# mayuelala/FollowYourClick

Measured on NVIDIA H100. Metric: frames/sec (64x64x16f latent, 25 DDIM steps), higher is better.
Workload: dtype bf16

## Files before the change

### followyourclick_b200/csrc/gemm_tc.cu

```cuda
#include "tma.cuh"
#include "wgmma.cuh"

namespace {

constexpr int BM = 128;
constexpr int BK = 64;
constexpr int STAGES = 4;
constexpr int A_BYTES = BM * BK * 2;
constexpr int MAX_STAGES = 8;
constexpr int MAX_RING_BYTES = 192 * 1024;
constexpr int SMEM_LIMIT = 232448;
constexpr int SMEM_EXTRA = 256 + 1024;
constexpr int OUT_BOX_BYTES = 32;
constexpr int OUT_BOX_SMEM = 64 * OUT_BOX_BYTES;
constexpr int NUM_THREADS = 288;

struct TcParams {
  int64_t M;
  int N, N_out;
  int taps, cin_blocks;
  int BN, n_tiles;
  int bw, bh, bn, Wo, Ho, w_tiles, h_tiles;
  int lg_bw, lg_bh;
  int64_t m_tiles;
  int tap_dy[9], tap_dx[9], tap_img[9];
  const float* bias; const float* rowbias;
  int64_t rows_per_group;
  int64_t ldrb;
  float alpha;
  int flags;
  int cb_split;
  const float* ln_rs;
  int resident, a_stages;
  int ring_bytes, stg_bytes;
  int half_dw, half_dh, half_dn;
};

__device__ __forceinline__ void warpgroup_sync(int wg) {
  if (wg == 0) asm volatile("bar.sync 1, 128;" ::: "memory");
  else asm volatile("bar.sync 2, 128;" ::: "memory");
}

struct TileCoord { int n, w, h, i; };
__device__ __forceinline__ TileCoord tile_coord(const TcParams& p, int64_t t) {
  TileCoord c;
  const uint32_t tile = (uint32_t)t;
  c.n = (int)(tile % (uint32_t)p.n_tiles);
  const uint32_t m_blk = tile / (uint32_t)p.n_tiles;
  c.w = (int)(m_blk % (uint32_t)p.w_tiles);
  const uint32_t m2 = m_blk / (uint32_t)p.w_tiles;
  c.h = (int)(m2 % (uint32_t)p.h_tiles);
  c.i = (int)(m2 / (uint32_t)p.h_tiles);
  return c;
}

__device__ __forceinline__ int64_t tile_pixel(const TcParams& p, const TileCoord& c, int r) {
  const int ow = c.w * p.bw + (r & (p.bw - 1)), oh = c.h * p.bh + ((r >> p.lg_bw) & (p.bh - 1));
  const int img = c.i * p.bn + (r >> (p.lg_bw + p.lg_bh));
  const int64_t pix = ((int64_t)img * p.Ho + oh) * p.Wo + ow;
  return ((ow < p.Wo) && (oh < p.Ho) && (pix < p.M)) ? pix : -1;
}

__device__ __forceinline__ uint32_t stage_off(int row, int col, int esize) {
  const int cpb = OUT_BOX_BYTES / esize;
  const uint32_t in_box = (uint32_t)(row * OUT_BOX_BYTES + (col % cpb) * esize);
  return (uint32_t)(col / cpb) * OUT_BOX_SMEM + (in_box ^ (((in_box >> 7) & 1u) << 4));
}

template <int BN, typename T>
__device__ __forceinline__ void epilogue(const TcParams& p, const TileCoord& c, const float* acc, int wg, int warp4, int lane, uint8_t* stg) {
  const int q = lane & 3;
  const int flags = p.flags;
  const bool geglu = flags & FYC_EPI_GEGLU, out_f32 = flags & FYC_EPI_OUT_F32, lnf = flags & FYC_EPI_LNFOLD;
  const bool has_bias = flags & FYC_EPI_BIAS, has_res = flags & FYC_EPI_RESIDUAL, has_rb = flags & FYC_EPI_ROWBIAS;
#pragma unroll
  for (int half = 0; half < 2; ++half) {
    const int row = warp4 * 16 + (lane >> 2) + 8 * half;
    const int64_t pix = tile_pixel(p, c, wg * 64 + row);
    if (pix < 0) continue;
    const float rs = lnf ? __ldg(p.ln_rs + pix) : 1.0f;
    const float* rb = has_rb ? p.rowbias + (pix / p.rows_per_group) * p.ldrb : nullptr;
    if (geglu) {
      if constexpr (BN == 256) {
        const float* bp = p.bias + c.n * 256;
#pragma unroll
        for (int j = 0; j < 16; ++j) {
          const int col = 8 * j + 2 * q;
          if (c.n * 128 + col >= p.N_out) continue;
          const float2 ba = __ldg(reinterpret_cast<const float2*>(bp + col)), bg = __ldg(reinterpret_cast<const float2*>(bp + 128 + col));
          const float a0 = acc[4 * j + 2 * half], a1 = acc[4 * j + 2 * half + 1];
          const float g0 = acc[4 * (j + 16) + 2 * half], g1 = acc[4 * (j + 16) + 2 * half + 1];
          const float x = fmaf(a0, rs, ba.x) * gelu_erf_fast(fmaf(g0, rs, bg.x));
          const float y = fmaf(a1, rs, ba.y) * gelu_erf_fast(fmaf(g1, rs, bg.y));
          *reinterpret_cast<typename Pair16<T>::type*>(stg + stage_off(row, col, 2)) = Pair16<T>::pack(x, y);
        }
      }
      continue;
    }
    const float scale = lnf ? rs : p.alpha;
#pragma unroll
    for (int j = 0; j < BN / 8; ++j) {
      const int col = 8 * j + 2 * q, n = c.n * BN + col;
      if (n >= p.N) continue;
      float x = acc[4 * j + 2 * half] * scale, y = acc[4 * j + 2 * half + 1] * scale;
      if (has_bias) { const float2 b = __ldg(reinterpret_cast<const float2*>(p.bias + n)); x += b.x; y += b.y; }
      if (has_rb) { const float2 b = __ldg(reinterpret_cast<const float2*>(rb + n)); x += b.x; y += b.y; }
      if (out_f32) {
        float2* s = reinterpret_cast<float2*>(stg + stage_off(row, col, 4));
        if (has_res) { const float2 r = *s; x += r.x; y += r.y; }
        *s = make_float2(x, y);
      } else {
        typename Pair16<T>::type* s = reinterpret_cast<typename Pair16<T>::type*>(stg + stage_off(row, col, 2));
        if (has_res) { const float2 r = Pair16<T>::unpack(*s); x += r.x; y += r.y; }
        *s = Pair16<T>::pack(x, y);
      }
    }
  }
}

template <int BN, typename T>
__global__ void __launch_bounds__(NUM_THREADS, 1)
gemm_tc_kernel(const __grid_constant__ CUtensorMap map_a, const __grid_constant__ CUtensorMap map_w, const __grid_constant__ CUtensorMap map_a2,
               const __grid_constant__ CUtensorMap map_out, const __grid_constant__ CUtensorMap map_res, const TcParams p) {
  extern __shared__ __align__(1024) uint8_t smem_raw[];
  uint8_t* smem = smem_raw + pad1024(smem_raw);
  uint64_t* bars = reinterpret_cast<uint64_t*>(smem + p.ring_bytes + 2 * p.stg_bytes);
  uint64_t* full = bars;
  uint64_t* empty = bars + MAX_STAGES;
  uint64_t* wbar = bars + 2 * MAX_STAGES;
  uint64_t* rbar = wbar + 1;
  const int nstages = p.a_stages;
  const uint32_t slab_kb = (uint32_t)BN * (BK * 2);
  const uint32_t a_base = p.resident ? (uint32_t)(p.taps * p.cin_blocks) * slab_kb : 0u;
  const uint32_t a_stride = p.resident ? (uint32_t)A_BYTES : (uint32_t)A_BYTES + slab_kb;
  const int warp = threadIdx.x >> 5, lane = threadIdx.x & 31;
  const int k_iters = p.taps * p.cin_blocks;
  const int64_t num_tiles = p.m_tiles * p.n_tiles;

  if (threadIdx.x == 0) {
    for (int s = 0; s < MAX_STAGES; ++s) { mbar_init(&full[s], 1); mbar_init(&empty[s], 256); }
    mbar_init(wbar, 1);
    mbar_init(&rbar[0], 1); mbar_init(&rbar[1], 1);
    mbar_init_fence();
  }
  __syncthreads();

  if (warp == 8) {
    if (lane == 0) {
      asm volatile("prefetch.tensormap [%0];" ::"l"(reinterpret_cast<uint64_t>(&map_a)) : "memory");
      asm volatile("prefetch.tensormap [%0];" ::"l"(reinterpret_cast<uint64_t>(&map_w)) : "memory");
      asm volatile("prefetch.tensormap [%0];" ::"l"(reinterpret_cast<uint64_t>(&map_a2)) : "memory");
      int stage = 0; uint32_t phase = 0;
      const uint32_t tx_bytes = p.resident ? (uint32_t)A_BYTES : A_BYTES + slab_kb;
      if (p.resident) {
        const int n_blk = (int)(blockIdx.x % p.n_tiles);
        mbar_expect_tx(wbar, (uint32_t)k_iters * slab_kb);
        for (int k = 0; k < k_iters; ++k)
          tma_load_3d(&map_w, wbar, smem + (uint32_t)k * slab_kb, (k % p.cin_blocks) * BK, k / p.cin_blocks, n_blk * BN);
      }
      for (int64_t tile = blockIdx.x; tile < num_tiles; tile += gridDim.x) {
        const TileCoord tc = tile_coord(p, tile);
        const int ow0 = tc.w * p.bw, oh0 = tc.h * p.bh, img0 = tc.i * p.bn;
        for (int tap = 0; tap < p.taps; ++tap) {
          for (int cb = 0; cb < p.cin_blocks; ++cb) {
            mbar_wait(&empty[stage], phase ^ 1);
            uint8_t* sa = smem + a_base + (uint32_t)stage * a_stride;
            const bool seg2 = cb >= p.cb_split;
            const CUtensorMap* ma = seg2 ? &map_a2 : &map_a;
            const int ka = (seg2 ? cb - p.cb_split : cb) * BK;
            mbar_expect_tx(&full[stage], tx_bytes);
            tma_load_4d(ma, &full[stage], sa, ka, ow0 + p.tap_dx[tap], oh0 + p.tap_dy[tap], img0 + p.tap_img[tap]);
            if (!p.resident) tma_load_3d(&map_w, &full[stage], sa + A_BYTES, cb * BK, tap, tc.n * BN);
            if (++stage == nstages) { stage = 0; phase ^= 1; }
          }
        }
      }
    }
    return;
  }
  const int wg = warp >> 2, warp4 = warp & 3;
  const bool elected = (threadIdx.x & 127) == 0;
  auto stg = [&]() { return smem + p.ring_bytes + wg * p.stg_bytes; };
  const bool has_res = p.flags & FYC_EPI_RESIDUAL;
  auto cpb = [&]() { return (p.flags & FYC_EPI_OUT_F32) ? OUT_BOX_BYTES / 4 : OUT_BOX_BYTES / 2; };
  if (elected) {
    asm volatile("prefetch.tensormap [%0];" ::"l"(reinterpret_cast<uint64_t>(&map_out)) : "memory");
    if (has_res) asm volatile("prefetch.tensormap [%0];" ::"l"(reinterpret_cast<uint64_t>(&map_res)) : "memory");
  }
  float acc[BN / 2];
  int stage = 0; uint32_t phase = 0, rphase = 0;
  if (p.resident) mbar_wait(wbar, 0);
  auto half_tile = [&](int64_t t, int& col0, int& nbox, int& bw0, int& bh0, int& bn0) {
    const TileCoord tc = tile_coord(p, t);
    const int bn_out = (p.flags & FYC_EPI_GEGLU) ? BN / 2 : BN;
    col0 = tc.n * bn_out;
    nbox = min(bn_out, p.N_out - col0) / cpb();
    bw0 = tc.w * p.bw + wg * p.half_dw; bh0 = tc.h * p.bh + wg * p.half_dh; bn0 = tc.i * p.bn + wg * p.half_dn;
    return tile_pixel(p, tc, wg * 64) >= 0;
  };
  for (int64_t tile = blockIdx.x; tile < num_tiles; tile += gridDim.x) {
    if (has_res && elected) {
      int col0, nbox, bw0, bh0, bn0;
      if (half_tile(tile, col0, nbox, bw0, bh0, bn0)) {
        bulk_wait_read();
        mbar_expect_tx(&rbar[wg], (uint32_t)(nbox * OUT_BOX_SMEM));
        for (int b = 0; b < nbox; ++b) tma_load_4d(&map_res, &rbar[wg], stg() + b * OUT_BOX_SMEM, col0 + b * cpb(), bw0, bh0, bn0);
      }
    }
    int prev = -1;
    for (int k = 0; k < k_iters; ++k) {
      mbar_wait(&full[stage], phase);
      const uint32_t sa = smem_u32(smem + a_base + (uint32_t)stage * a_stride) + (uint32_t)wg * (64 * BK * 2);
      const uint64_t a_desc = wgmma_desc_sw128(sa);
      const uint64_t b_desc = wgmma_desc_sw128(p.resident ? smem_u32(smem) + (uint32_t)k * slab_kb : smem_u32(smem + (uint32_t)stage * a_stride) + A_BYTES);
      wgmma_fence();
#pragma unroll
      for (int kk = 0; kk < BK / 16; ++kk)
        Wgmma<BN, T>::ss(acc, a_desc + (uint64_t)(2 * kk), b_desc + (uint64_t)(2 * kk), (k > 0 || kk > 0) ? 1 : 0);
      wgmma_commit();
      wgmma_wait<1>();
      if (prev >= 0) mbar_arrive(&empty[prev]);
      prev = stage;
      if (++stage == nstages) { stage = 0; phase ^= 1; }
    }
    wgmma_wait<0>();
    wgmma_fence_regs<BN / 2>(acc);
    mbar_arrive(&empty[prev]);
    int col0, nbox, bw0, bh0, bn0;
    if (!half_tile(tile, col0, nbox, bw0, bh0, bn0)) continue;
    if (elected) bulk_wait_read();
    warpgroup_sync(wg);
    if (has_res) { mbar_wait(&rbar[wg], rphase); rphase ^= 1; }
    epilogue<BN, T>(p, tile_coord(p, tile), acc, wg, warp4, lane, stg());
    fence_async_smem();
    warpgroup_sync(wg);
    if (elected) {
      for (int b = 0; b < nbox; ++b) tma_store_4d(&map_out, stg() + b * OUT_BOX_SMEM, col0 + b * cpb(), bw0, bh0, bn0);
      bulk_commit();
    }
  }
  if (elected) bulk_wait_all();
}

__global__ void space_to_planes_kernel(const bf16* __restrict__ x, bf16* __restrict__ out, int64_t NB, int64_t H, int64_t W, int64_t C) {
  const int64_t cv = C / 8, H2 = H / 2, W2 = W / 2;
  const int64_t total = NB * H * W * cv;
  for (int64_t i = blockIdx.x * (int64_t)blockDim.x + threadIdx.x; i < total; i += (int64_t)gridDim.x * blockDim.x) {
    int64_t c = (i % cv) * 8; int64_t t = i / cv;
    int64_t w = t % W; t /= W;
    int64_t h = t % H; int64_t n = t / H;
    int64_t plane = 2 * (h & 1) + (w & 1);
    bf16* dst = out + ((((plane * NB + n) * H2) + h / 2) * W2 + w / 2) * C + c;
    *reinterpret_cast<uint4*>(dst) = *reinterpret_cast<const uint4*>(x + i * 8);
  }
}

int32_t encode_out_map(CUtensorMap* m, const void* base, const TcParams& p, int32_t dt, uint64_t cols, uint64_t W, uint64_t H, uint64_t NB,
                       uint64_t sw, uint64_t sh, uint64_t sn) {
  const bool f32 = (p.flags & FYC_EPI_OUT_F32) != 0;
  const uint64_t es = f32 ? 4 : 2;
  uint64_t dims[4] = {cols, W, H, NB};
  uint64_t str[3] = {sw * es, sh * es, sn * es};
  uint32_t box[4] = {(uint32_t)(OUT_BOX_BYTES / es), (uint32_t)(p.half_dw ? p.half_dw : p.bw), (uint32_t)(p.half_dh ? p.half_dh : p.bh),
                     (uint32_t)(p.half_dn ? p.half_dn : p.bn)};
  return encode_map(m, base, 4, dims, str, box, f32 ? CU_TENSOR_MAP_DATA_TYPE_FLOAT32 : tma_dtype(dt),
                    CU_TENSOR_MAP_SWIZZLE_32B);
}

constexpr int BN_CHOICES[] = {256, 192, 160, 128, 96, 80, 64, 48, 32, 16};
constexpr int MAX_BN_F32 = 128;

int pick_bn(int64_t N, bool geglu, bool f32) {
  if (geglu) return 256;
  for (int bn : BN_CHOICES)
    if (N % bn == 0 && (!f32 || bn <= MAX_BN_F32)) return bn;
  return 16;
}

int stg_bytes_for(int bn, int flags) {
  const int bn_out = (flags & FYC_EPI_GEGLU) ? bn / 2 : bn;
  return 64 * bn_out * ((flags & FYC_EPI_OUT_F32) ? 4 : 2);
}
int ring_bytes_for(int bn, int flags) {
  const int avail = (SMEM_LIMIT - SMEM_EXTRA - 2 * stg_bytes_for(bn, flags)) & ~1023;
  return avail < MAX_RING_BYTES ? avail : MAX_RING_BYTES;
}

void choose_tiles(TcParams& p, int* grid_out) {
  const int sms = fyc_sm_count();
  const bool geglu = (p.flags & FYC_EPI_GEGLU) != 0, f32 = (p.flags & FYC_EPI_OUT_F32) != 0;
  const int max_bn = f32 ? MAX_BN_F32 : 256;
  const int k_iters = p.taps * p.cin_blocks;
  p.resident = 0;
  p.BN = pick_bn(p.N, geglu, f32);
  p.n_tiles = (int)ceil_div64(p.N, p.BN);
  p.half_dw = p.half_dh = p.half_dn = 0;
  if (p.bn >= 2) p.half_dn = p.bn / 2;
  else if (p.bh >= 2) p.half_dh = p.bh / 2;
  else p.half_dw = p.bw / 2;
  int grid = 0;
  if (!geglu) {
    int rbn = 0;
    for (int min_stages = 4; min_stages >= 3 && !rbn; --min_stages)
      for (int bn : BN_CHOICES)
        if (bn >= 128 && bn <= max_bn && p.N % bn == 0 &&
            (int64_t)k_iters * bn * 128 <= ring_bytes_for(bn, p.flags) - min_stages * A_BYTES) { rbn = bn; break; }
    if (rbn) {
      const int nt = p.N / rbn;
      const int rgrid = (sms / nt) * nt;
      if (nt <= sms && rgrid * 16 >= sms * 15 && p.m_tiles * nt >= (int64_t)rgrid * 4) {
        p.resident = 1; p.BN = rbn; p.n_tiles = nt;
        grid = rgrid;
      }
    }
    const int64_t rounds0 = ceil_div64(p.m_tiles * p.n_tiles, sms);
    if (!p.resident && rounds0 < 8) {
      auto cost_of = [&](int bn, int64_t nt) {
        const int64_t mma = 8 * bn, feed = (int64_t)(5.3 * (128 + bn));
        return ceil_div64(p.m_tiles * nt, sms) * ((mma > feed ? mma : feed) + 400);
      };
      int64_t best = cost_of(p.BN, p.n_tiles);
      for (int bn : BN_CHOICES) {
        if (bn > p.N || bn < 64 || bn > max_bn) continue;
        const int64_t nt = ceil_div64(p.N, bn);
        const int64_t cost = cost_of(bn, nt);
        if (cost < best) { best = cost; p.BN = bn; p.n_tiles = (int)nt; }
      }
    }
  }
  p.stg_bytes = stg_bytes_for(p.BN, p.flags);
  p.ring_bytes = ring_bytes_for(p.BN, p.flags);
  const int slab = k_iters * p.BN * 128;
  const int st = p.resident ? (p.ring_bytes - slab) / A_BYTES : p.ring_bytes / (A_BYTES + p.BN * 128);
  p.a_stages = st > (p.resident ? MAX_STAGES : STAGES) ? (p.resident ? MAX_STAGES : STAGES) : st;
  if (!p.resident) {
    const int64_t tiles = p.m_tiles * p.n_tiles;
    grid = (int)(tiles < sms ? tiles : sms);
  }
  *grid_out = grid;
}

template <int BN, typename T>
int32_t launch_bn(const CUtensorMap& ma, const CUtensorMap& mw, const CUtensorMap& ma2, const CUtensorMap& mo, const CUtensorMap& mr,
                  const TcParams& p, int grid, cudaStream_t st) {
  static bool attr_set = false;
  if (!attr_set) {
    FYC_CUDA(cudaFuncSetAttribute(gemm_tc_kernel<BN, T>, cudaFuncAttributeMaxDynamicSharedMemorySize, SMEM_LIMIT));
    attr_set = true;
  }
  const int smem = p.ring_bytes + 2 * p.stg_bytes + SMEM_EXTRA;
  FYC_CHECK(smem <= SMEM_LIMIT && p.a_stages >= 2 && p.a_stages <= MAX_STAGES, "tensor-core GEMM: shared-memory plan does not fit (BN %d)", BN);
  gemm_tc_kernel<BN, T><<<grid, NUM_THREADS, smem, st>>>(ma, mw, ma2, mo, mr, p);
  FYC_LAUNCH_CHECK();
  return FYC_OK;
}

int32_t launch_tc(int32_t dt, const CUtensorMap& ma, const CUtensorMap& mw, const CUtensorMap& mo, const CUtensorMap* mr, TcParams p, int grid,
                  cudaStream_t st, const CUtensorMap* ma2p = nullptr) {
  const CUtensorMap& ma2 = ma2p ? *ma2p : ma;
  const CUtensorMap& mres = mr ? *mr : mo;
  if (!ma2p) p.cb_split = 0x7fffffff;
  FYC_CHECK(!(p.flags & FYC_EPI_RESIDUAL) || mr, "tensor-core GEMM: residual epilogue without a residual map");
  FYC_CHECK((p.bw & (p.bw - 1)) == 0 && (p.bh & (p.bh - 1)) == 0 && p.bw > 0 && p.bh > 0, "tensor-core GEMM: patch dims must be powers of two");
  p.lg_bw = 0; while ((1 << p.lg_bw) < p.bw) ++p.lg_bw;
  p.lg_bh = 0; while ((1 << p.lg_bh) < p.bh) ++p.lg_bh;
  const int64_t tiles = p.m_tiles * p.n_tiles;
  FYC_CHECK(tiles < (1ll << 31) && p.M < (1ll << 31) && p.rows_per_group < (1ll << 31), "tensor-core GEMM: problem exceeds the 32-bit tile index range");
  if (grid > tiles) grid = (int)tiles;
  FYC_DISPATCH16(dt, switch (p.BN) {
    case 256: return launch_bn<256, T>(ma, mw, ma2, mo, mres, p, grid, st);
    case 192: return launch_bn<192, T>(ma, mw, ma2, mo, mres, p, grid, st);
    case 160: return launch_bn<160, T>(ma, mw, ma2, mo, mres, p, grid, st);
    case 128: return launch_bn<128, T>(ma, mw, ma2, mo, mres, p, grid, st);
    case 96: return launch_bn<96, T>(ma, mw, ma2, mo, mres, p, grid, st);
    case 80: return launch_bn<80, T>(ma, mw, ma2, mo, mres, p, grid, st);
    case 64: return launch_bn<64, T>(ma, mw, ma2, mo, mres, p, grid, st);
    case 48: return launch_bn<48, T>(ma, mw, ma2, mo, mres, p, grid, st);
    case 32: return launch_bn<32, T>(ma, mw, ma2, mo, mres, p, grid, st);
    case 16: return launch_bn<16, T>(ma, mw, ma2, mo, mres, p, grid, st);
  })
  FYC_CHECK(false, "tensor-core GEMM: no kernel for BN = %d", p.BN);
}

}

bool fyc_gemm_tc_eligible(const fyc_gemm_args* g) {
  if (!fyc_is_16bit(g->dtype)) return false;
  if (g->K % 8 || g->lda % 8 || g->ldw % 8 || g->N % 16 || g->M < 64) return false;
  if (((uintptr_t)g->A | (uintptr_t)g->W) & 15) return false;
  if (g->batch > 1 && ((g->strideA | g->strideW | g->strideO) % 8)) return false;
  const int64_t n_out = (g->epilogue & FYC_EPI_GEGLU) ? g->N / 2 : g->N;
  if (g->ldo % 8 || ((uintptr_t)g->out & 15)) return false;
  if ((g->epilogue & FYC_EPI_RESIDUAL) && (g->ldr % 8 || ((uintptr_t)g->residual & 15))) return false;
  if ((g->epilogue & FYC_EPI_GEGLU) && (g->N % 256 || !(g->epilogue & FYC_EPI_BIAS) || (g->epilogue & ~(FYC_EPI_GEGLU | FYC_EPI_BIAS | FYC_EPI_LNFOLD)))) return false;
  if (g->A2) {
    if (g->batch != 1 || g->K1 <= 0 || g->K1 >= g->K || g->K1 % BK || g->lda2 % 8 || (((uintptr_t)g->A2) & 15)) return false;
  }
  if (g->epilogue & FYC_EPI_LNFOLD) {
    if (!g->ln_rowstats || (((uintptr_t)g->ln_rowstats) & 3)) return false;
    if (g->alpha != 1.0f || (g->epilogue & (FYC_EPI_OUT_F32 | FYC_EPI_RESIDUAL)) || g->N % 8) return false;
    if ((g->epilogue & FYC_EPI_ROWBIAS) && g->rows_per_group % 128) return false;
  }
  if ((g->epilogue & FYC_EPI_BIAS) && ((uintptr_t)g->bias & 15)) return false;
  if ((g->epilogue & FYC_EPI_ROWBIAS) && ((uintptr_t)g->rowbias & 15)) return false;
  (void)n_out;
  return tma_available();
}

int32_t fyc_gemm_tc(const fyc_gemm_args* g, cudaStream_t st) {
  FYC_CHECK(fyc_gemm_tc_eligible(g), "gemm(tensor cores): shape/alignment not eligible (M=%lld N=%lld K=%lld)", (long long)g->M,
            (long long)g->N, (long long)g->K);
  const bool geglu = (g->epilogue & FYC_EPI_GEGLU) != 0;
  const bool f32 = (g->epilogue & FYC_EPI_OUT_F32) != 0;
  for (int64_t b = 0; b < g->batch; ++b) {
    const uint16_t* A = (const uint16_t*)g->A + b * g->strideA;
    const uint16_t* W = (const uint16_t*)g->W + b * g->strideW;
    CUtensorMap ma, mw, ma2;
    const int64_t Ka = g->A2 ? g->K1 : g->K;
    {
      uint64_t dims[4] = {(uint64_t)Ka, (uint64_t)g->M, 1, 1};
      uint64_t str[3] = {(uint64_t)g->lda * 2, (uint64_t)g->lda * 2 * (uint64_t)g->M, (uint64_t)g->lda * 2 * (uint64_t)g->M};
      uint32_t box[4] = {BK, BM, 1, 1};
      int32_t rc = encode_map(&ma, A, 4, dims, str, box, tma_dtype(g->dtype));
      if (rc) return rc;
    }
    if (g->A2) {
      uint64_t dims[4] = {(uint64_t)(g->K - g->K1), (uint64_t)g->M, 1, 1};
      uint64_t str[3] = {(uint64_t)g->lda2 * 2, (uint64_t)g->lda2 * 2 * (uint64_t)g->M, (uint64_t)g->lda2 * 2 * (uint64_t)g->M};
      uint32_t box[4] = {BK, BM, 1, 1};
      int32_t rc = encode_map(&ma2, g->A2, 4, dims, str, box, tma_dtype(g->dtype));
      if (rc) return rc;
    }
    TcParams p{};
    p.M = g->M; p.N = (int)g->N; p.N_out = geglu ? (int)g->N / 2 : (int)g->N;
    p.taps = 1; p.cin_blocks = (int)ceil_div64(g->K, BK);
    p.bw = BM; p.bh = 1; p.bn = 1; p.Wo = (int)g->M; p.Ho = 1;
    p.w_tiles = (int)ceil_div64(g->M, BM); p.h_tiles = 1; p.m_tiles = p.w_tiles;
    p.flags = g->epilogue;
    int grid = 0;
    choose_tiles(p, &grid);
    p.tap_dy[0] = p.tap_dx[0] = p.tap_img[0] = 0;
    {
      uint64_t dims[3] = {(uint64_t)g->K, 1, (uint64_t)g->N};
      uint64_t str[2] = {(uint64_t)g->ldw * 2, (uint64_t)g->ldw * 2};
      uint32_t box[3] = {BK, 1, (uint32_t)p.BN};
      int32_t rc = encode_map(&mw, W, 3, dims, str, box, tma_dtype(g->dtype));
      if (rc) return rc;
    }
    FYC_CHECK(g->M < (1ll << 31), "gemm(tensor cores): M too large");
    p.bias = g->bias; p.rowbias = g->rowbias; p.rows_per_group = g->rows_per_group > 0 ? g->rows_per_group : 1; p.ldrb = g->N;
    p.alpha = g->alpha;
    p.ln_rs = g->ln_rowstats;
    p.cb_split = g->A2 ? (int)(g->K1 / BK) : 0x7fffffff;
    const int64_t es = f32 ? 4 : 2;
    const uint64_t M = (uint64_t)g->M, No = (uint64_t)p.N_out;
    CUtensorMap mo, mr;
    int32_t rc = encode_out_map(&mo, (const char*)g->out + b * g->strideO * es, p, g->dtype, No, M, 1, 1, g->ldo, g->ldo * M, g->ldo * M);
    if (rc) return rc;
    if (g->epilogue & FYC_EPI_RESIDUAL) {
      rc = encode_out_map(&mr, (const char*)g->residual + b * g->strideO * es, p, g->dtype, No, M, 1, 1, g->ldr, g->ldr * M, g->ldr * M);
      if (rc) return rc;
    }
    rc = launch_tc(g->dtype, ma, mw, mo, (g->epilogue & FYC_EPI_RESIDUAL) ? &mr : nullptr, p, grid, st, g->A2 ? &ma2 : nullptr);
    if (rc) return rc;
  }
  return FYC_OK;
}

static bool pick_patch(int64_t NB, int64_t Ho, int64_t Wo, int* bw, int* bh, int* bn) {
  int w = 1; while (w < 128 && Wo % (w * 2) == 0) w *= 2;
  int h = 1; while (w * h < 128 && Ho % (h * 2) == 0) h *= 2;
  int n = 128 / (w * h);
  if (w * h * n != 128 || NB % n != 0) return false;
  *bw = w; *bh = h; *bn = n;
  return true;
}

bool fyc_conv3x3_tc_eligible(const fyc_conv3x3_args* c) {
  if (!fyc_is_16bit(c->dtype) || c->upsample != 1) return false;
  if (c->stride != 1 && c->stride != 2) return false;
  if (c->Cin % 8 || c->Cout % 16) return false;
  if (c->stride == 2 && (c->H % 2 || c->W % 2)) return false;
  if (((uintptr_t)c->x | (uintptr_t)c->w | (uintptr_t)c->out) & 15) return false;
  if ((c->epilogue & FYC_EPI_RESIDUAL) && ((uintptr_t)c->residual & 15)) return false;
  if ((c->epilogue & FYC_EPI_ROWBIAS) && (((uintptr_t)c->rowbias & 15) || (c->ld_rowbias > 0 && c->ld_rowbias % 4))) return false;
  if (c->epilogue & FYC_EPI_GEGLU) return false;
  int bw, bh, bn;
  if (!pick_patch(c->NB, c->H / c->stride, c->W / c->stride, &bw, &bh, &bn)) return false;
  return tma_available();
}

int32_t fyc_conv3x3_tc(const fyc_conv3x3_args* c, const void* x_planes, cudaStream_t st) {
  FYC_CHECK(fyc_conv3x3_tc_eligible(c), "conv3x3(tensor cores): shape/alignment not eligible");
  const int s = c->stride;
  const int64_t Ho = c->H / s, Wo = c->W / s;
  TcParams p{};
  pick_patch(c->NB, Ho, Wo, &p.bw, &p.bh, &p.bn);
  p.M = c->NB * Ho * Wo; p.N = (int)c->Cout; p.N_out = p.N;
// ... 115 lines not shown
```

### followyourclick_b200/csrc/wgmma.cuh

```cuda
#pragma once
#include <stdint.h>

#include "common.cuh"

template <int N, typename T = bf16> struct Wgmma;

#define FYC_WGMMA_16(T, TY) \
template <> struct Wgmma<16, T> { \
  static __device__ __forceinline__ void ss(float* d, uint64_t da, uint64_t db, int scale_d) { \
    asm volatile("{\n.reg .pred p;\nsetp.ne.b32 p, %10, 0;\n" \
                 "wgmma.mma_async.sync.aligned.m64n16k16.f32." TY "." TY " {%0, %1, %2, %3, %4, %5, %6, %7}, %8, %9, p, 1, 1, 0, 0;\n}" \
                 : "+f"(d[0]), "+f"(d[1]), "+f"(d[2]), "+f"(d[3]), "+f"(d[4]), "+f"(d[5]), "+f"(d[6]), "+f"(d[7]) \
                 : "l"(da), "l"(db), "r"(scale_d)); \
  } \
};
FYC_WGMMA_16(bf16, "bf16")
FYC_WGMMA_16(f16, "f16")
#undef FYC_WGMMA_16

#define FYC_WGMMA_32(T, TY) \
template <> struct Wgmma<32, T> { \
  static __device__ __forceinline__ void ss(float* d, uint64_t da, uint64_t db, int scale_d) { \
    asm volatile("{\n.reg .pred p;\nsetp.ne.b32 p, %18, 0;\n" \
                 "wgmma.mma_async.sync.aligned.m64n32k16.f32." TY "." TY " {%0, %1, %2, %3, %4, %5, %6, %7, %8, %9, %10, %11, %12, %13, %14, %15}, %16, %17, p, 1, 1, 0, 0;\n}" \
// ... 85 lines not shown
  } \
};
FYC_WGMMA_128(bf16, "bf16")
FYC_WGMMA_128(f16, "f16")
#undef FYC_WGMMA_128

#define FYC_WGMMA_160(T, TY) \
template <> struct Wgmma<160, T> { \
  static __device__ __forceinline__ void ss(float* d, uint64_t da, uint64_t db, int scale_d) { \
    asm volatile("{\n.reg .pred p;\nsetp.ne.b32 p, %82, 0;\n" \
                 "wgmma.mma_async.sync.aligned.m64n160k16.f32." TY "." TY " {%0, %1, %2, %3, %4, %5, %6, %7, %8, %9, %10, %11, %12, %13, %14, %15, %16, %17, %18, %19, %20, %21, %22, %23, %24, %25, %26, %27, %28, %29, %30, %31, %32, %33, %34, %35, %36, %37, %38, %39, %40, %41, %42, %43, %44, %45, %46, %47, %48, %49, %50, %51, %52, %53, %54, %55, %56, %57, %58, %59, %60, %61, %62, %63, %64, %65, %66, %67, %68, %69, %70, %71, %72, %73, %74, %75, %76, %77, %78, %79}, %80, %81, p, 1, 1, 0, 0;\n}" \
                 : "+f"(d[0]), "+f"(d[1]), "+f"(d[2]), "+f"(d[3]), "+f"(d[4]), "+f"(d[5]), "+f"(d[6]), "+f"(d[7]), "+f"(d[8]), "+f"(d[9]), "+f"(d[10]), "+f"(d[11]), "+f"(d[12]), "+f"(d[13]), "+f"(d[14]), "+f"(d[15]), "+f"(d[16]), "+f"(d[17]), "+f"(d[18]), "+f"(d[19]), "+f"(d[20]), "+f"(d[21]), "+f"(d[22]), "+f"(d[23]), "+f"(d[24]), "+f"(d[25]), "+f"(d[26]), "+f"(d[27]), "+f"(d[28]), "+f"(d[29]), "+f"(d[30]), "+f"(d[31]), "+f"(d[32]), "+f"(d[33]), "+f"(d[34]), "+f"(d[35]), "+f"(d[36]), "+f"(d[37]), "+f"(d[38]), "+f"(d[39]), "+f"(d[40]), "+f"(d[41]), "+f"(d[42]), "+f"(d[43]), "+f"(d[44]), "+f"(d[45]), "+f"(d[46]), "+f"(d[47]), "+f"(d[48]), "+f"(d[49]), "+f"(d[50]), "+f"(d[51]), "+f"(d[52]), "+f"(d[53]), "+f"(d[54]), "+f"(d[55]), "+f"(d[56]), "+f"(d[57]), "+f"(d[58]), "+f"(d[59]), "+f"(d[60]), "+f"(d[61]), "+f"(d[62]), "+f"(d[63]), "+f"(d[64]), "+f"(d[65]), "+f"(d[66]), "+f"(d[67]), "+f"(d[68]), "+f"(d[69]), "+f"(d[70]), "+f"(d[71]), "+f"(d[72]), "+f"(d[73]), "+f"(d[74]), "+f"(d[75]), "+f"(d[76]), "+f"(d[77]), "+f"(d[78]), "+f"(d[79]) \
                 : "l"(da), "l"(db), "r"(scale_d)); \
  } \
};
FYC_WGMMA_160(bf16, "bf16")
FYC_WGMMA_160(f16, "f16")
#undef FYC_WGMMA_160

#define FYC_WGMMA_192(T, TY) \
template <> struct Wgmma<192, T> { \
  static __device__ __forceinline__ void ss(float* d, uint64_t da, uint64_t db, int scale_d) { \
    asm volatile("{\n.reg .pred p;\nsetp.ne.b32 p, %98, 0;\n" \
                 "wgmma.mma_async.sync.aligned.m64n192k16.f32." TY "." TY " {%0, %1, %2, %3, %4, %5, %6, %7, %8, %9, %10, %11, %12, %13, %14, %15, %16, %17, %18, %19, %20, %21, %22, %23, %24, %25, %26, %27, %28, %29, %30, %31, %32, %33, %34, %35, %36, %37, %38, %39, %40, %41, %42, %43, %44, %45, %46, %47, %48, %49, %50, %51, %52, %53, %54, %55, %56, %57, %58, %59, %60, %61, %62, %63, %64, %65, %66, %67, %68, %69, %70, %71, %72, %73, %74, %75, %76, %77, %78, %79, %80, %81, %82, %83, %84, %85, %86, %87, %88, %89, %90, %91, %92, %93, %94, %95}, %96, %97, p, 1, 1, 0, 0;\n}" \
                 : "+f"(d[0]), "+f"(d[1]), "+f"(d[2]), "+f"(d[3]), "+f"(d[4]), "+f"(d[5]), "+f"(d[6]), "+f"(d[7]), "+f"(d[8]), "+f"(d[9]), "+f"(d[10]), "+f"(d[11]), "+f"(d[12]), "+f"(d[13]), "+f"(d[14]), "+f"(d[15]), "+f"(d[16]), "+f"(d[17]), "+f"(d[18]), "+f"(d[19]), "+f"(d[20]), "+f"(d[21]), "+f"(d[22]), "+f"(d[23]), "+f"(d[24]), "+f"(d[25]), "+f"(d[26]), "+f"(d[27]), "+f"(d[28]), "+f"(d[29]), "+f"(d[30]), "+f"(d[31]), "+f"(d[32]), "+f"(d[33]), "+f"(d[34]), "+f"(d[35]), "+f"(d[36]), "+f"(d[37]), "+f"(d[38]), "+f"(d[39]), "+f"(d[40]), "+f"(d[41]), "+f"(d[42]), "+f"(d[43]), "+f"(d[44]), "+f"(d[45]), "+f"(d[46]), "+f"(d[47]), "+f"(d[48]), "+f"(d[49]), "+f"(d[50]), "+f"(d[51]), "+f"(d[52]), "+f"(d[53]), "+f"(d[54]), "+f"(d[55]), "+f"(d[56]), "+f"(d[57]), "+f"(d[58]), "+f"(d[59]), "+f"(d[60]), "+f"(d[61]), "+f"(d[62]), "+f"(d[63]), "+f"(d[64]), "+f"(d[65]), "+f"(d[66]), "+f"(d[67]), "+f"(d[68]), "+f"(d[69]), "+f"(d[70]), "+f"(d[71]), "+f"(d[72]), "+f"(d[73]), "+f"(d[74]), "+f"(d[75]), "+f"(d[76]), "+f"(d[77]), "+f"(d[78]), "+f"(d[79]), "+f"(d[80]), "+f"(d[81]), "+f"(d[82]), "+f"(d[83]), "+f"(d[84]), "+f"(d[85]), "+f"(d[86]), "+f"(d[87]), "+f"(d[88]), "+f"(d[89]), "+f"(d[90]), "+f"(d[91]), "+f"(d[92]), "+f"(d[93]), "+f"(d[94]), "+f"(d[95]) \
                 : "l"(da), "l"(db), "r"(scale_d)); \
  } \
};
FYC_WGMMA_192(bf16, "bf16")
FYC_WGMMA_192(f16, "f16")
#undef FYC_WGMMA_192

#define FYC_WGMMA_256(T, TY) \
template <> struct Wgmma<256, T> { \
  static __device__ __forceinline__ void ss(float* d, uint64_t da, uint64_t db, int scale_d) { \
    asm volatile("{\n.reg .pred p;\nsetp.ne.b32 p, %130, 0;\n" \
                 "wgmma.mma_async.sync.aligned.m64n256k16.f32." TY "." TY " {%0, %1, %2, %3, %4, %5, %6, %7, %8, %9, %10, %11, %12, %13, %14, %15, %16, %17, %18, %19, %20, %21, %22, %23, %24, %25, %26, %27, %28, %29, %30, %31, %32, %33, %34, %35, %36, %37, %38, %39, %40, %41, %42, %43, %44, %45, %46, %47, %48, %49, %50, %51, %52, %53, %54, %55, %56, %57, %58, %59, %60, %61, %62, %63, %64, %65, %66, %67, %68, %69, %70, %71, %72, %73, %74, %75, %76, %77, %78, %79, %80, %81, %82, %83, %84, %85, %86, %87, %88, %89, %90, %91, %92, %93, %94, %95, %96, %97, %98, %99, %100, %101, %102, %103, %104, %105, %106, %107, %108, %109, %110, %111, %112, %113, %114, %115, %116, %117, %118, %119, %120, %121, %122, %123, %124, %125, %126, %127}, %128, %129, p, 1, 1, 0, 0;\n}" \
                 : "+f"(d[0]), "+f"(d[1]), "+f"(d[2]), "+f"(d[3]), "+f"(d[4]), "+f"(d[5]), "+f"(d[6]), "+f"(d[7]), "+f"(d[8]), "+f"(d[9]), "+f"(d[10]), "+f"(d[11]), "+f"(d[12]), "+f"(d[13]), "+f"(d[14]), "+f"(d[15]), "+f"(d[16]), "+f"(d[17]), "+f"(d[18]), "+f"(d[19]), "+f"(d[20]), "+f"(d[21]), "+f"(d[22]), "+f"(d[23]), "+f"(d[24]), "+f"(d[25]), "+f"(d[26]), "+f"(d[27]), "+f"(d[28]), "+f"(d[29]), "+f"(d[30]), "+f"(d[31]), "+f"(d[32]), "+f"(d[33]), "+f"(d[34]), "+f"(d[35]), "+f"(d[36]), "+f"(d[37]), "+f"(d[38]), "+f"(d[39]), "+f"(d[40]), "+f"(d[41]), "+f"(d[42]), "+f"(d[43]), "+f"(d[44]), "+f"(d[45]), "+f"(d[46]), "+f"(d[47]), "+f"(d[48]), "+f"(d[49]), "+f"(d[50]), "+f"(d[51]), "+f"(d[52]), "+f"(d[53]), "+f"(d[54]), "+f"(d[55]), "+f"(d[56]), "+f"(d[57]), "+f"(d[58]), "+f"(d[59]), "+f"(d[60]), "+f"(d[61]), "+f"(d[62]), "+f"(d[63]), "+f"(d[64]), "+f"(d[65]), "+f"(d[66]), "+f"(d[67]), "+f"(d[68]), "+f"(d[69]), "+f"(d[70]), "+f"(d[71]), "+f"(d[72]), "+f"(d[73]), "+f"(d[74]), "+f"(d[75]), "+f"(d[76]), "+f"(d[77]), "+f"(d[78]), "+f"(d[79]), "+f"(d[80]), "+f"(d[81]), "+f"(d[82]), "+f"(d[83]), "+f"(d[84]), "+f"(d[85]), "+f"(d[86]), "+f"(d[87]), "+f"(d[88]), "+f"(d[89]), "+f"(d[90]), "+f"(d[91]), "+f"(d[92]), "+f"(d[93]), "+f"(d[94]), "+f"(d[95]), "+f"(d[96]), "+f"(d[97]), "+f"(d[98]), "+f"(d[99]), "+f"(d[100]), "+f"(d[101]), "+f"(d[102]), "+f"(d[103]), "+f"(d[104]), "+f"(d[105]), "+f"(d[106]), "+f"(d[107]), "+f"(d[108]), "+f"(d[109]), "+f"(d[110]), "+f"(d[111]), "+f"(d[112]), "+f"(d[113]), "+f"(d[114]), "+f"(d[115]), "+f"(d[116]), "+f"(d[117]), "+f"(d[118]), "+f"(d[119]), "+f"(d[120]), "+f"(d[121]), "+f"(d[122]), "+f"(d[123]), "+f"(d[124]), "+f"(d[125]), "+f"(d[126]), "+f"(d[127]) \
                 : "l"(da), "l"(db), "r"(scale_d)); \
  } \
};
FYC_WGMMA_256(bf16, "bf16")
FYC_WGMMA_256(f16, "f16")
#undef FYC_WGMMA_256

__device__ __forceinline__ void wgmma_fence() { asm volatile("wgmma.fence.sync.aligned;" ::: "memory"); }
__device__ __forceinline__ void wgmma_commit() { asm volatile("wgmma.commit_group.sync.aligned;" ::: "memory"); }
template <int N> __device__ __forceinline__ void wgmma_wait() { asm volatile("wgmma.wait_group.sync.aligned %0;" ::"n"(N) : "memory"); }
template <int NR> __device__ __forceinline__ void wgmma_fence_regs(float* d) {
#pragma unroll
  for (int i = 0; i < NR; ++i) asm volatile("" : "+f"(d[i])::"memory");
}

__device__ __forceinline__ uint64_t wgmma_desc_sw128(uint32_t saddr) {
  uint64_t d = 0;
  d |= (uint64_t)((saddr & 0x3FFFF) >> 4);
  d |= (uint64_t)1 << 16;
  d |= (uint64_t)(1024 >> 4) << 32;
  d |= (uint64_t)1 << 62;
  return d;
}
```

Baseline: 6.125.

## Switch tensor-core GEMM to ping-pong consumer warpgroups with register reallocation

Restructures the warp-specialized GEMM so each consumer warpgroup computes a whole 128-row tile, and the two warpgroups alternate tiles under ordered named barriers. One group's epilogue then overlaps the other's MMA main loop. It adds a producer warpgroup with setmaxnreg to shift registers to the consumers, caps BN at 192 (64 for f32), and interleaves GEGLU weight rows in 16-row TMA boxes so GEGLU can use BN 128/160 and resident weights. The risks are higher register pressure from doubling the accumulators, more TMA issues for GEGLU weights, and changed tile-choice heuristics.

```diff
diff --git a/followyourclick_b200/csrc/gemm_tc.cu b/followyourclick_b200/csrc/gemm_tc.cu
--- a/followyourclick_b200/csrc/gemm_tc.cu
+++ b/followyourclick_b200/csrc/gemm_tc.cu
@@ -12,8 +12,10 @@
 constexpr int SMEM_LIMIT = 232448;
 constexpr int SMEM_EXTRA = 256 + 1024;
 constexpr int OUT_BOX_BYTES = 32;
-constexpr int OUT_BOX_SMEM = 64 * OUT_BOX_BYTES;
-constexpr int NUM_THREADS = 288;
+constexpr int OUT_BOX_SMEM = BM * OUT_BOX_BYTES;
+constexpr int NUM_THREADS = 384;
+constexpr int PRODUCER_REGS = 40, CONSUMER_REGS = 232;
+constexpr int GEGLU_BOX = 16;
 
 struct TcParams {
   int64_t M;
@@ -33,12 +35,19 @@
   const float* ln_rs;
   int resident, a_stages;
   int ring_bytes, stg_bytes;
-  int half_dw, half_dh, half_dn;
 };
 
 __device__ __forceinline__ void warpgroup_sync(int wg) {
   if (wg == 0) asm volatile("bar.sync 1, 128;" ::: "memory");
   else asm volatile("bar.sync 2, 128;" ::: "memory");
+}
+__device__ __forceinline__ void order_wait(int wg) {
+  if (wg == 0) asm volatile("bar.sync 3, 256;" ::: "memory");
+  else asm volatile("bar.sync 4, 256;" ::: "memory");
+}
+__device__ __forceinline__ void order_arrive(int wg) {
+  if (wg == 0) asm volatile("bar.arrive 3, 256;" ::: "memory");
+  else asm volatile("bar.arrive 4, 256;" ::: "memory");
 }
 
 struct TileCoord { int n, w, h, i; };
@@ -61,6 +70,8 @@
   return ((ow < p.Wo) && (oh < p.Ho) && (pix < p.M)) ? pix : -1;
 }
 
+__device__ __forceinline__ int geglu_row(int v) { return 256 * (v >> 7) + (v & 127); }
+
 __device__ __forceinline__ uint32_t stage_off(int row, int col, int esize) {
   const int cpb = OUT_BOX_BYTES / esize;
   const uint32_t in_box = (uint32_t)(row * OUT_BOX_BYTES + (col % cpb) * esize);
@@ -68,51 +79,56 @@
 }
 
 template <int BN, typename T>
-__device__ __forceinline__ void epilogue(const TcParams& p, const TileCoord& c, const float* acc, int wg, int warp4, int lane, uint8_t* stg) {
+__device__ __forceinline__ void epilogue(const TcParams& p, const TileCoord& c, const float* acc, int warp4, int lane, uint8_t* stg) {
   const int q = lane & 3;
   const int flags = p.flags;
   const bool geglu = flags & FYC_EPI_GEGLU, out_f32 = flags & FYC_EPI_OUT_F32, lnf = flags & FYC_EPI_LNFOLD;
   const bool has_bias = flags & FYC_EPI_BIAS, has_res = flags & FYC_EPI_RESIDUAL, has_rb = flags & FYC_EPI_ROWBIAS;
 #pragma unroll
-  for (int half = 0; half < 2; ++half) {
-    const int row = warp4 * 16 + (lane >> 2) + 8 * half;
-    const int64_t pix = tile_pixel(p, c, wg * 64 + row);
-    if (pix < 0) continue;
-    const float rs = lnf ? __ldg(p.ln_rs + pix) : 1.0f;
-    const float* rb = has_rb ? p.rowbias + (pix / p.rows_per_group) * p.ldrb : nullptr;
-    if (geglu) {
-      if constexpr (BN == 256) {
-        const float* bp = p.bias + c.n * 256;
+  for (int mh = 0; mh < 2; ++mh) {
+    const float* a = acc + mh * (BN / 2);
 #pragma unroll
-        for (int j = 0; j < 16; ++j) {
-          const int col = 8 * j + 2 * q;
-          if (c.n * 128 + col >= p.N_out) continue;
-          const float2 ba = __ldg(reinterpret_cast<const float2*>(bp + col)), bg = __ldg(reinterpret_cast<const float2*>(bp + 128 + col));
-          const float a0 = acc[4 * j + 2 * half], a1 = acc[4 * j + 2 * half + 1];
-          const float g0 = acc[4 * (j + 16) + 2 * half], g1 = acc[4 * (j + 16) + 2 * half + 1];
-          const float x = fmaf(a0, rs, ba.x) * gelu_erf_fast(fmaf(g0, rs, bg.x));
-          const float y = fmaf(a1, rs, ba.y) * gelu_erf_fast(fmaf(g1, rs, bg.y));
-          *reinterpret_cast<typename Pair16<T>::type*>(stg + stage_off(row, col, 2)) = Pair16<T>::pack(x, y);
+    for (int half = 0; half < 2; ++half) {
+      const int row = mh * 64 + warp4 * 16 + (lane >> 2) + 8 * half;
+      const int64_t pix = tile_pixel(p, c, row);
+      if (pix < 0) continue;
+      const float rs = lnf ? __ldg(p.ln_rs + pix) : 1.0f;
+      const float* rb = has_rb ? p.rowbias + (pix / p.rows_per_group) * p.ldrb : nullptr;
+      if (geglu) {
+        if constexpr (BN % (2 * GEGLU_BOX) == 0) {
+          constexpr int HJ = BN / 16;
+#pragma unroll
+          for (int j = 0; j < HJ; ++j) {
+            const int col = 8 * j + 2 * q, v = c.n * (BN / 2) + col;
+            if (v >= p.N_out) continue;
+            const float* bp = p.bias + geglu_row(v & ~15) + (v & 15);
+            const float2 ba = __ldg(reinterpret_cast<const float2*>(bp)), bg = __ldg(reinterpret_cast<const float2*>(bp + 128));
+            const float a0 = a[4 * j + 2 * half], a1 = a[4 * j + 2 * half + 1];
+            const float g0 = a[4 * (j + HJ) + 2 * half], g1 = a[4 * (j + HJ) + 2 * half + 1];
+            const float x = fmaf(a0, rs, ba.x) * gelu_erf_fast(fmaf(g0, rs, bg.x));
+            const float y = fmaf(a1, rs, ba.y) * gelu_erf_fast(fmaf(g1, rs, bg.y));
+            *reinterpret_cast<typename Pair16<T>::type*>(stg + stage_off(row, col, 2)) = Pair16<T>::pack(x, y);
+          }
         }
+        continue;
       }
-      continue;
-    }
-    const float scale = lnf ? rs : p.alpha;
+      const float scale = lnf ? rs : p.alpha;
 #pragma unroll
-    for (int j = 0; j < BN / 8; ++j) {
-      const int col = 8 * j + 2 * q, n = c.n * BN + col;
-      if (n >= p.N) continue;
-      float x = acc[4 * j + 2 * half] * scale, y = acc[4 * j + 2 * half + 1] * scale;
-      if (has_bias) { const float2 b = __ldg(reinterpret_cast<const float2*>(p.bias + n)); x += b.x; y += b.y; }
-      if (has_rb) { const float2 b = __ldg(reinterpret_cast<const float2*>(rb + n)); x += b.x; y += b.y; }
-      if (out_f32) {
-        float2* s = reinterpret_cast<float2*>(stg + stage_off(row, col, 4));
-        if (has_res) { const float2 r = *s; x += r.x; y += r.y; }
-        *s = make_float2(x, y);
-      } else {
-        typename Pair16<T>::type* s = reinterpret_cast<typename Pair16<T>::type*>(stg + stage_off(row, col, 2));
-        if (has_res) { const float2 r = Pair16<T>::unpack(*s); x += r.x; y += r.y; }
-        *s = Pair16<T>::pack(x, y);
+      for (int j = 0; j < BN / 8; ++j) {
+        const int col = 8 * j + 2 * q, n = c.n * BN + col;
+        if (n >= p.N) continue;
+        float x = a[4 * j + 2 * half] * scale, y = a[4 * j + 2 * half + 1] * scale;
+        if (has_bias) { const float2 b = __ldg(reinterpret_cast<const float2*>(p.bias + n)); x += b.x; y += b.y; }
+        if (has_rb) { const float2 b = __ldg(reinterpret_cast<const float2*>(rb + n)); x += b.x; y += b.y; }
+        if (out_f32) {
+          float2* s = reinterpret_cast<float2*>(stg + stage_off(row, col, 4));
+          if (has_res) { const float2 r = *s; x += r.x; y += r.y; }
+          *s = make_float2(x, y);
+        } else {
+          typename Pair16<T>::type* s = reinterpret_cast<typename Pair16<T>::type*>(stg + stage_off(row, col, 2));
+          if (has_res) { const float2 r = Pair16<T>::unpack(*s); x += r.x; y += r.y; }
+          *s = Pair16<T>::pack(x, y);
+        }
       }
     }
   }
@@ -136,27 +152,37 @@
   const int warp = threadIdx.x >> 5, lane = threadIdx.x & 31;
   const int k_iters = p.taps * p.cin_blocks;
   const int64_t num_tiles = p.m_tiles * p.n_tiles;
+  const int n_mine = (int)((num_tiles - 1 - blockIdx.x) / gridDim.x) + 1;
 
   if (threadIdx.x == 0) {
-    for (int s = 0; s < MAX_STAGES; ++s) { mbar_init(&full[s], 1); mbar_init(&empty[s], 256); }
+    for (int s = 0; s < MAX_STAGES; ++s) { mbar_init(&full[s], 1); mbar_init(&empty[s], 128); }
     mbar_init(wbar, 1);
     mbar_init(&rbar[0], 1); mbar_init(&rbar[1], 1);
     mbar_init_fence();
   }
   __syncthreads();
 
-  if (warp == 8) {
-    if (lane == 0) {
+  if (warp >= 8) {
+    setmaxnreg_dec<PRODUCER_REGS>();
+    if (warp == 8 && lane == 0) {
       asm volatile("prefetch.tensormap [%0];" ::"l"(reinterpret_cast<uint64_t>(&map_a)) : "memory");
       asm volatile("prefetch.tensormap [%0];" ::"l"(reinterpret_cast<uint64_t>(&map_w)) : "memory");
       asm volatile("prefetch.tensormap [%0];" ::"l"(reinterpret_cast<uint64_t>(&map_a2)) : "memory");
+      const bool geglu = p.flags & FYC_EPI_GEGLU;
+      auto load_w = [&](uint64_t* bar, uint8_t* dst, int kc, int tap, int n_blk) {
+        if (!geglu) { tma_load_3d(&map_w, bar, dst, kc, tap, n_blk * BN); return; }
+        for (int b = 0; b < BN / (2 * GEGLU_BOX); ++b) {
+          const int row = geglu_row(n_blk * (BN / 2) + b * GEGLU_BOX);
+          tma_load_3d(&map_w, bar, dst + b * (GEGLU_BOX * BK * 2), kc, tap, row);
+          tma_load_3d(&map_w, bar, dst + (BN / 2 + b * GEGLU_BOX) * (BK * 2), kc, tap, row + 128);
+        }
+      };
       int stage = 0; uint32_t phase = 0;
       const uint32_t tx_bytes = p.resident ? (uint32_t)A_BYTES : A_BYTES + slab_kb;
       if (p.resident) {
         const int n_blk = (int)(blockIdx.x % p.n_tiles);
         mbar_expect_tx(wbar, (uint32_t)k_iters * slab_kb);
-        for (int k = 0; k < k_iters; ++k)
-          tma_load_3d(&map_w, wbar, smem + (uint32_t)k * slab_kb, (k % p.cin_blocks) * BK, k / p.cin_blocks, n_blk * BN);
+        for (int k = 0; k < k_iters; ++k) load_w(wbar, smem + (uint32_t)k * slab_kb, (k % p.cin_blocks) * BK, k / p.cin_blocks, n_blk);
       }
       for (int64_t tile = blockIdx.x; tile < num_tiles; tile += gridDim.x) {
         const TileCoord tc = tile_coord(p, tile);
@@ -170,7 +196,7 @@
             const int ka = (seg2 ? cb - p.cb_split : cb) * BK;
             mbar_expect_tx(&full[stage], tx_bytes);
             tma_load_4d(ma, &full[stage], sa, ka, ow0 + p.tap_dx[tap], oh0 + p.tap_dy[tap], img0 + p.tap_img[tap]);
-            if (!p.resident) tma_load_3d(&map_w, &full[stage], sa + A_BYTES, cb * BK, tap, tc.n * BN);
+            if (!p.resident) load_w(&full[stage], sa + A_BYTES, cb * BK, tap, tc.n);
             if (++stage == nstages) { stage = 0; phase ^= 1; }
           }
         }
@@ -178,64 +204,68 @@
     }
     return;
   }
+  setmaxnreg_inc<CONSUMER_REGS>();
   const int wg = warp >> 2, warp4 = warp & 3;
+  if (wg >= n_mine) return;
   const bool elected = (threadIdx.x & 127) == 0;
-  auto stg = [&]() { return smem + p.ring_bytes + wg * p.stg_bytes; };
+  uint8_t* const stg = smem + p.ring_bytes + wg * p.stg_bytes;
   const bool has_res = p.flags & FYC_EPI_RESIDUAL;
-  auto cpb = [&]() { return (p.flags & FYC_EPI_OUT_F32) ? OUT_BOX_BYTES / 4 : OUT_BOX_BYTES / 2; };
+  const int cpb = (p.flags & FYC_EPI_OUT_F32) ? OUT_BOX_BYTES / 4 : OUT_BOX_BYTES / 2;
+  const int bn_out = (p.flags & FYC_EPI_GEGLU) ? BN / 2 : BN;
   if (elected) {
     asm volatile("prefetch.tensormap [%0];" ::"l"(reinterpret_cast<uint64_t>(&map_out)) : "memory");
     if (has_res) asm volatile("prefetch.tensormap [%0];" ::"l"(reinterpret_cast<uint64_t>(&map_res)) : "memory");
   }
-  float acc[BN / 2];
-  int stage = 0; uint32_t phase = 0, rphase = 0;
+  float acc[BN];
+  uint32_t rphase = 0;
   if (p.resident) mbar_wait(wbar, 0);
-  auto half_tile = [&](int64_t t, int& col0, int& nbox, int& bw0, int& bh0, int& bn0) {
-    const TileCoord tc = tile_coord(p, t);
-    const int bn_out = (p.flags & FYC_EPI_GEGLU) ? BN / 2 : BN;
-    col0 = tc.n * bn_out;
-    nbox = min(bn_out, p.N_out - col0) / cpb();
-    bw0 = tc.w * p.bw + wg * p.half_dw; bh0 = tc.h * p.bh + wg * p.half_dh; bn0 = tc.i * p.bn + wg * p.half_dn;
-    return tile_pixel(p, tc, wg * 64) >= 0;
-  };
-  for (int64_t tile = blockIdx.x; tile < num_tiles; tile += gridDim.x) {
+  for (int j = wg; j < n_mine; j += 2) {
+    const int64_t tile = blockIdx.x + (int64_t)j * gridDim.x;
     if (has_res && elected) {
-      int col0, nbox, bw0, bh0, bn0;
-      if (half_tile(tile, col0, nbox, bw0, bh0, bn0)) {
-        bulk_wait_read();
-        mbar_expect_tx(&rbar[wg], (uint32_t)(nbox * OUT_BOX_SMEM));
-        for (int b = 0; b < nbox; ++b) tma_load_4d(&map_res, &rbar[wg], stg() + b * OUT_BOX_SMEM, col0 + b * cpb(), bw0, bh0, bn0);
-      }
-    }
+      const TileCoord tc = tile_coord(p, tile);
+      const int col0 = tc.n * bn_out, nbox = min(bn_out, p.N_out - col0) / cpb;
+      bulk_wait_read();
+      mbar_expect_tx(&rbar[wg], (uint32_t)(nbox * OUT_BOX_SMEM));
+      for (int b = 0; b < nbox; ++b)
+        tma_load_4d(&map_res, &rbar[wg], stg + b * OUT_BOX_SMEM, col0 + b * cpb, tc.w * p.bw, tc.h * p.bh, tc.i * p.bn);
+    }
+    const uint32_t pos0 = (uint32_t)j * (uint32_t)k_iters;
+    int stage = (int)(pos0 % (uint32_t)nstages);
+    uint32_t phase = (pos0 / (uint32_t)nstages) & 1u;
+    if (j > 0) order_wait(wg);
     int prev = -1;
     for (int k = 0; k < k_iters; ++k) {
       mbar_wait(&full[stage], phase);
-      const uint32_t sa = smem_u32(smem + a_base + (uint32_t)stage * a_stride) + (uint32_t)wg * (64 * BK * 2);
-      const uint64_t a_desc = wgmma_desc_sw128(sa);
-      const uint64_t b_desc = wgmma_desc_sw128(p.resident ? smem_u32(smem) + (uint32_t)k * slab_kb : smem_u32(smem + (uint32_t)stage * a_stride) + A_BYTES);
+      const uint32_t sa = smem_u32(smem + a_base + (uint32_t)stage * a_stride);
+      const uint64_t a_lo = wgmma_desc_sw128(sa), a_hi = wgmma_desc_sw128(sa + 64 * BK * 2);
+      const uint64_t b_desc = wgmma_desc_sw128(p.resident ? smem_u32(smem) + (uint32_t)k * slab_kb : sa + A_BYTES);
       wgmma_fence();
 #pragma unroll
-      for (int kk = 0; kk < BK / 16; ++kk)
-        Wgmma<BN, T>::ss(acc, a_desc + (uint64_t)(2 * kk), b_desc + (uint64_t)(2 * kk), (k > 0 || kk > 0) ? 1 : 0);
+      for (int kk = 0; kk < BK / 16; ++kk) {
+        const int acc_in = (k > 0 || kk > 0) ? 1 : 0;
+        Wgmma<BN, T>::ss(acc, a_lo + (uint64_t)(2 * kk), b_desc + (uint64_t)(2 * kk), acc_in);
+        Wgmma<BN, T>::ss(acc + BN / 2, a_hi + (uint64_t)(2 * kk), b_desc + (uint64_t)(2 * kk), acc_in);
+      }
       wgmma_commit();
       wgmma_wait<1>();
       if (prev >= 0) mbar_arrive(&empty[prev]);
       prev = stage;
       if (++stage == nstages) { stage = 0; phase ^= 1; }
     }
+    if (j + 1 < n_mine) order_arrive(wg ^ 1);
     wgmma_wait<0>();
-    wgmma_fence_regs<BN / 2>(acc);
+    wgmma_fence_regs<BN>(acc);
     mbar_arrive(&empty[prev]);
-    int col0, nbox, bw0, bh0, bn0;
-    if (!half_tile(tile, col0, nbox, bw0, bh0, bn0)) continue;
+    const TileCoord tc = tile_coord(p, tile);
     if (elected) bulk_wait_read();
     warpgroup_sync(wg);
     if (has_res) { mbar_wait(&rbar[wg], rphase); rphase ^= 1; }
-    epilogue<BN, T>(p, tile_coord(p, tile), acc, wg, warp4, lane, stg());
+    epilogue<BN, T>(p, tc, acc, warp4, lane, stg);
     fence_async_smem();
     warpgroup_sync(wg);
     if (elected) {
-      for (int b = 0; b < nbox; ++b) tma_store_4d(&map_out, stg() + b * OUT_BOX_SMEM, col0 + b * cpb(), bw0, bh0, bn0);
+      const int col0 = tc.n * bn_out, nbox = min(bn_out, p.N_out - col0) / cpb;
+      for (int b = 0; b < nbox; ++b) tma_store_4d(&map_out, stg + b * OUT_BOX_SMEM, col0 + b * cpb, tc.w * p.bw, tc.h * p.bh, tc.i * p.bn);
       bulk_commit();
     }
   }
@@ -261,17 +291,16 @@
   const uint64_t es = f32 ? 4 : 2;
   uint64_t dims[4] = {cols, W, H, NB};
   uint64_t str[3] = {sw * es, sh * es, sn * es};
-  uint32_t box[4] = {(uint32_t)(OUT_BOX_BYTES / es), (uint32_t)(p.half_dw ? p.half_dw : p.bw), (uint32_t)(p.half_dh ? p.half_dh : p.bh),
-                     (uint32_t)(p.half_dn ? p.half_dn : p.bn)};
+  uint32_t box[4] = {(uint32_t)(OUT_BOX_BYTES / es), (uint32_t)p.bw, (uint32_t)p.bh, (uint32_t)p.bn};
   return encode_map(m, base, 4, dims, str, box, f32 ? CU_TENSOR_MAP_DATA_TYPE_FLOAT32 : tma_dtype(dt),
                     CU_TENSOR_MAP_SWIZZLE_32B);
 }
 
-constexpr int BN_CHOICES[] = {256, 192, 160, 128, 96, 80, 64, 48, 32, 16};
-constexpr int MAX_BN_F32 = 128;
+constexpr int BN_CHOICES[] = {192, 160, 128, 96, 80, 64, 48, 32, 16};
+constexpr int MAX_BN_F32 = 64;
 
 int pick_bn(int64_t N, bool geglu, bool f32) {
-  if (geglu) return 256;
+  if (geglu) return (N / 2) % 80 == 0 ? 160 : 128;
   for (int bn : BN_CHOICES)
     if (N % bn == 0 && (!f32 || bn <= MAX_BN_F32)) return bn;
   return 16;
@@ -279,53 +308,47 @@
 
 int stg_bytes_for(int bn, int flags) {
   const int bn_out = (flags & FYC_EPI_GEGLU) ? bn / 2 : bn;
-  return 64 * bn_out * ((flags & FYC_EPI_OUT_F32) ? 4 : 2);
+  return BM * bn_out * ((flags & FYC_EPI_OUT_F32) ? 4 : 2);
 }
 int ring_bytes_for(int bn, int flags) {
   const int avail = (SMEM_LIMIT - SMEM_EXTRA - 2 * stg_bytes_for(bn, flags)) & ~1023;
   return avail < MAX_RING_BYTES ? avail : MAX_RING_BYTES;
 }
 
+int64_t plain_cost(int64_t m_tiles, int bn, int64_t nt, int k_iters, int sms) {
+  const int64_t mma = 8 * bn, feed = (int64_t)(5.3 * (128 + bn));
+  return ceil_div64(m_tiles * nt, sms) * k_iters * (mma > feed ? mma : feed);
+}
+
 void choose_tiles(TcParams& p, int* grid_out) {
   const int sms = fyc_sm_count();
   const bool geglu = (p.flags & FYC_EPI_GEGLU) != 0, f32 = (p.flags & FYC_EPI_OUT_F32) != 0;
-  const int max_bn = f32 ? MAX_BN_F32 : 256;
+  const int max_bn = f32 ? MAX_BN_F32 : 192;
   const int k_iters = p.taps * p.cin_blocks;
   p.resident = 0;
   p.BN = pick_bn(p.N, geglu, f32);
   p.n_tiles = (int)ceil_div64(p.N, p.BN);
-  p.half_dw = p.half_dh = p.half_dn = 0;
-  if (p.bn >= 2) p.half_dn = p.bn / 2;
-  else if (p.bh >= 2) p.half_dh = p.bh / 2;
-  else p.half_dw = p.bw / 2;
   int grid = 0;
-  if (!geglu) {
-    int rbn = 0;
-    for (int min_stages = 4; min_stages >= 3 && !rbn; --min_stages)
-      for (int bn : BN_CHOICES)
-        if (bn >= 128 && bn <= max_bn && p.N % bn == 0 &&
-            (int64_t)k_iters * bn * 128 <= ring_bytes_for(bn, p.flags) - min_stages * A_BYTES) { rbn = bn; break; }
-    if (rbn) {
-      const int nt = p.N / rbn;
-      const int rgrid = (sms / nt) * nt;
-      if (nt <= sms && rgrid * 16 >= sms * 15 && p.m_tiles * nt >= (int64_t)rgrid * 4) {
-        p.resident = 1; p.BN = rbn; p.n_tiles = nt;
-        grid = rgrid;
-      }
-    }
-    const int64_t rounds0 = ceil_div64(p.m_tiles * p.n_tiles, sms);
-    if (!p.resident && rounds0 < 8) {
-      auto cost_of = [&](int bn, int64_t nt) {
-        const int64_t mma = 8 * bn, feed = (int64_t)(5.3 * (128 + bn));
-        return ceil_div64(p.m_tiles * nt, sms) * ((mma > feed ? mma : feed) + 400);
-      };
-      int64_t best = cost_of(p.BN, p.n_tiles);
-      for (int bn : BN_CHOICES) {
-        if (bn > p.N || bn < 64 || bn > max_bn) continue;
-        const int64_t nt = ceil_div64(p.N, bn);
-        const int64_t cost = cost_of(bn, nt);
-        if (cost < best) { best = cost; p.BN = bn; p.n_tiles = (int)nt; }
-      }
+  int rbn = 0;
+  for (int min_stages = 4; min_stages >= 3 && !rbn; --min_stages)
+    for (int bn : BN_CHOICES)
+      if (bn >= 128 && bn <= max_bn && (!geglu || bn == p.BN) && p.N % bn == 0 &&
+          (int64_t)k_iters * bn * 128 <= ring_bytes_for(bn, p.flags) - min_stages * A_BYTES) { rbn = bn; break; }
+  if (rbn) {
+    const int nt = p.N / rbn;
+    const int rgrid = (sms / nt) * nt;
+    if (nt <= sms && rgrid * 16 >= sms * 15 && p.m_tiles * nt >= (int64_t)rgrid * 4) {
+      p.resident = 1; p.BN = rbn; p.n_tiles = nt;
+      grid = rgrid;
+    }
+  }
+  if (!geglu && !p.resident && ceil_div64(p.m_tiles * p.n_tiles, sms) < 8) {
+    int64_t best = plain_cost(p.m_tiles, p.BN, p.n_tiles, k_iters, sms);
+    for (int bn : BN_CHOICES) {
+      if (bn > p.N || bn < 64 || bn > max_bn) continue;
+      const int64_t nt = ceil_div64(p.N, bn);
+      const int64_t cost = plain_cost(p.m_tiles, bn, nt, k_iters, sms);
+      if (cost < best) { best = cost; p.BN = bn; p.n_tiles = (int)nt; }
     }
   }
   p.stg_bytes = stg_bytes_for(p.BN, p.flags);
@@ -368,7 +391,6 @@
   FYC_CHECK(tiles < (1ll << 31) && p.M < (1ll << 31) && p.rows_per_group < (1ll << 31), "tensor-core GEMM: problem exceeds the 32-bit tile index range");
   if (grid > tiles) grid = (int)tiles;
   FYC_DISPATCH16(dt, switch (p.BN) {
-    case 256: return launch_bn<256, T>(ma, mw, ma2, mo, mres, p, grid, st);
     case 192: return launch_bn<192, T>(ma, mw, ma2, mo, mres, p, grid, st);
     case 160: return launch_bn<160, T>(ma, mw, ma2, mo, mres, p, grid, st);
     case 128: return launch_bn<128, T>(ma, mw, ma2, mo, mres, p, grid, st);
@@ -443,7 +465,7 @@
     {
       uint64_t dims[3] = {(uint64_t)g->K, 1, (uint64_t)g->N};
       uint64_t str[2] = {(uint64_t)g->ldw * 2, (uint64_t)g->ldw * 2};
-      uint32_t box[3] = {BK, 1, (uint32_t)p.BN};
+      uint32_t box[3] = {BK, 1, (uint32_t)(geglu ? GEGLU_BOX : p.BN)};
       int32_t rc = encode_map(&mw, W, 3, dims, str, box, tma_dtype(g->dtype));
       if (rc) return rc;
     }
diff --git a/followyourclick_b200/csrc/wgmma.cuh b/followyourclick_b200/csrc/wgmma.cuh
--- a/followyourclick_b200/csrc/wgmma.cuh
+++ b/followyourclick_b200/csrc/wgmma.cuh
@@ -161,6 +161,9 @@
   for (int i = 0; i < NR; ++i) asm volatile("" : "+f"(d[i])::"memory");
 }
 
+template <int R> __device__ __forceinline__ void setmaxnreg_inc() { asm volatile("setmaxnreg.inc.sync.aligned.u32 %0;" ::"n"(R)); }
+template <int R> __device__ __forceinline__ void setmaxnreg_dec() { asm volatile("setmaxnreg.dec.sync.aligned.u32 %0;" ::"n"(R)); }
+
 __device__ __forceinline__ uint64_t wgmma_desc_sw128(uint32_t saddr) {
   uint64_t d = 0;
   d |= (uint64_t)((saddr & 0x3FFFF) >> 4);
```

New measurement: 6.274, median of 6. 1.02x the previous value.
